# SonyResearch/micro_diffusion

Hardware: AMD Instinct MI355X
Metric: training images/sec (global batch 2048) MicroDiT-XL/2 256-res mask=0.75 (higher is better)
Workload: dtype bf16; 1 GPU; MicroDiT_XL_2 res_256_pretrain.yaml mask=0.75, full step = 2 microbatches x 1024 fwd+bwd + grad exchange + clip 0.25 + AdamW; global_batch=2048, microbatch=1024, parallelism=dp1, grad_exchange=none (single rank)

## Files before the change

### micro_diffusion_amd/csrc/gemm.hip

```cpp
#include "md_common.h"
#include "gemm_common.h"
#include <stdlib.h>

namespace {

constexpr int BM = 128, BN = 128;
constexpr int PITCH_KC = (BKT + 8) * 2;
constexpr int PITCH_KS = (BM + 32) * 2;
constexpr int TILE_BYTES = (BM * PITCH_KC > BKT * PITCH_KS) ? BM * PITCH_KC : BKT * PITCH_KS;
constexpr int SLAB_PITCH = 68;
constexpr int SLAB_FLOATS = 32 * SLAB_PITCH;
static_assert(4 * SLAB_FLOATS * 4 <= 2 * TILE_BYTES, "epilogue slab must fit in the staging LDS");

typedef __attribute__((address_space(3))) s16x4 lds_s16x4;

__device__ __forceinline__ bf16x4 lds_tr_read(const unsigned char* p) {
    s16x4 v = __builtin_amdgcn_ds_read_tr16_b64_v4i16((lds_s16x4*)(p));
    U64 t;
    t.s = v;
    return t.h;
}

__device__ __forceinline__ void tile_coords(int bid, int nwg, int ntn, int group_n, int& tm, int& tn) {
    const int q = nwg >> 3, r = nwg & 7, xcd = bid & 7, j = bid >> 3;
// ... 531 lines not shown
            w4 = md_gemm_w4_fills(t * a->ksplit, a->cu_limit);
        }
        if (a->chosen_variant) *a->chosen_variant = w4 ? MD_GEMM_W4 : MD_GEMM_PP256;
        return w4 ? md_gemm_w4_launch(a, stream) : md_gemm_pp_launch(a, stream);
    }
    if (!a->A || !a->B || !a->C) return MD_BAD_ARG;
    if (a->M <= 0 || a->N <= 0 || a->K <= 0 || a->batch <= 0 || a->ksplit <= 0) return MD_BAD_ARG;
    if (a->lda % 8 || a->ldb % 8) return MD_BAD_ARG;
    if ((a->mode == MD_EPI_STORE_BF16 || a->mode == MD_EPI_RESIDUAL || a->mode == MD_EPI_DACT || a->mode == MD_EPI_SWIGLU_BWD) ? (a->ldc % 8) : (a->ldc % 4))
        return MD_BAD_ARG;
    if (a->C2 && a->ldc2 % 8) return MD_BAD_ARG;
    if (a->ksplit > 1 && !(a->mode == MD_EPI_ATOMIC_F32 || (a->mode == MD_EPI_STORE_F32 && a->sSplit > 0))) return MD_BAD_ARG;
    if (a->mode == MD_EPI_RESIDUAL && (!a->res || (a->gate && a->rows_per_sample <= 0))) return MD_BAD_ARG;
    if (a->mode == MD_EPI_DACT && !a->aux) return MD_BAD_ARG;
    if (a->mode < MD_EPI_STORE_BF16 || a->mode > MD_EPI_SWIGLU_BWD) return MD_BAD_ARG;
    if (a->mode == MD_EPI_SWIGLU_BWD) {
        if (!a->aux || a->ldaux % 8) return MD_BAD_ARG;
        if (a->variant != MD_GEMM_AUTO && a->variant != MD_GEMM_W4) return MD_NOT_ELIGIBLE;
        if (!md_gemm_w4_eligible(a) || (a->cu_limit > 0 && a->cu_limit < 256) || getenv("MD_GEMM_NO_W4")) return MD_NOT_ELIGIBLE;
        a_copy.variant = MD_GEMM_W4;
    }
    if (a->dact_cached && (a->act != MD_ACT_GELU_ERF || !(a->mode == MD_EPI_DACT || (a->mode == MD_EPI_STORE_BF16 && a->C2)))) return MD_BAD_ARG;
    const int64_t tiles256 = ((a->M + 255) / 256) * ((a->N + 255) / 256) * (int64_t)a->batch * a->ksplit;
    const int64_t kspan = (a->K + a->ksplit - 1) / a->ksplit;
    int variant = a->variant;
    if (variant < MD_GEMM_AUTO || variant > MD_GEMM_W4) return MD_BAD_ARG;
    if (variant == MD_GEMM_PP256 && !md_gemm_pp_eligible(a)) return MD_NOT_ELIGIBLE;
    if (variant == MD_GEMM_W4 && !md_gemm_w4_eligible(a)) return MD_NOT_ELIGIBLE;
    if ((a->A_list || a->B_list) && !(a->A_list && a->B_list && md_gemm_pp_eligible(a))) return MD_BAD_ARG;
    if (a->A_list) variant = MD_GEMM_PP256;
    if (variant == MD_GEMM_AUTO) {
        const char* w4min = getenv("MD_GEMM_W4_MIN_TILES");
        if (md_gemm_w4_eligible(a) && tiles256 >= (w4min ? atoi(w4min) : 192) && md_gemm_w4_fills(tiles256, a->cu_limit) && !getenv("MD_GEMM_NO_W4") &&
            (a->a_kcontig || !getenv("MD_GEMM_NO_W4_TN")))
            variant = MD_GEMM_W4;
        else if (md_gemm_pp_eligible(a) && tiles256 >= 192)
            variant = MD_GEMM_PP256;
        else if (!a->a_kcontig && !a->b_kcontig && kspan >= 2048 && tiles256 >= 128)
            variant = MD_GEMM_PACED256;
        else if (a->K >= 1024 && tiles256 >= 224 && tiles256 <= 256)
            variant = MD_GEMM_PACED256;
        else if (kspan > 2048 && tiles256 >= 240 && (tiles256 % 256 == 0 || tiles256 % 256 >= 160 || tiles256 >= 2048))
            variant = MD_GEMM_PACED256;
        else if (a->a_kcontig && a->K <= 2048)
            variant = MD_GEMM_REG128;
        else
            variant = ((!a->a_kcontig && !a->b_kcontig) || a->K < 1024) ? MD_GEMM_REG128 : MD_GEMM_DMA128;
// ... 32 lines not shown
```

### micro_diffusion_amd/csrc/gemm_pp.hip

```cpp
#include "gemm_pp_common.h"

namespace {

constexpr bool pp_is_dact(int epi) { return epi == PP_E_DACT_GELU || epi == PP_E_DACT_MUL; }
constexpr bool pp_is_gelu(int epi) { return epi == PP_E_BF16_GELU || epi == PP_E_BF16_GELU_D; }

template <int EPI>
__device__ __forceinline__ int epi_prefetch_count(const md_gemm_args& p) {
    if (EPI == PP_E_RES) return p.gate ? 5 : 4;
    if (pp_is_dact(EPI)) return 4;
    return 0;
}

template <int EPI, int IH, int JH>
__device__ __forceinline__ void epi_prefetch(const md_gemm_args& p, const PPPlan& w, const EpiTile& et, u32x4 (&pre)[5],
                                             const EpiLane& el) {
    const unsigned ld = EPI == PP_E_RES ? (unsigned)p.ldr : (unsigned)p.ldaux;
    const int mlast = w.M - 1 - et.m0;
    const int nlast = ((w.N - 1) & ~7) - et.n0;
    int rq, cq;
    el.quad_coords(rq, cq);
    const int c = cq + JH * 128;
    const unsigned coff = (unsigned)(c < nlast ? c : nlast);
#pragma unroll
// ... 168 lines not shown
template <int AKC, int BKC, int EPI>
__global__ __launch_bounds__(512) void gemm_bf16_pp_kernel(md_gemm_args p, PPPlan w) {
    __shared__ __attribute__((aligned(1024))) unsigned char smem[2 * B_REGION];
    const int tid = threadIdx.x, lane = tid & 63;
    const int wave = __builtin_amdgcn_readfirstlane(tid >> 6);
    const int wr = wave >> 2, wc = wave & 3;

    constexpr bool TAILABLE = EPI != PP_E_F32;
    int w_first, w_stride, w_count;
    {
        const int G = gridDim.x, x = blockIdx.x & 7, j = blockIdx.x >> 3;
        const int body = (TAILABLE && w.tail_units) ? w.tail_first : w.total;
        const int q = body >> 3, r = body & 7;
        const int lo = x < r ? x * (q + 1) : r * (q + 1) + (x - r) * q;
        const int cnt = q + (x < r ? 1 : 0);
        w_stride = (G - x + 7) >> 3;
        w_first = lo + j;
        w_count = j < cnt ? (int)((unsigned)(cnt - j + w_stride - 1) / (unsigned)w_stride) : 0;
    }
    const int tail_n = (TAILABLE && (int)blockIdx.x < w.tail_units) ? w_count : -1;
    if (w_count == 0 && tail_n < 0) return;
    long long* const tl = p.timeline ? static_cast<long long*>(p.timeline) + (size_t)blockIdx.x * 16 : nullptr;
    if (tl && tid == 0) { tl[0] = clock64(); tl[1] = wall_clock64(); }
    const int half_iters = w_count * (w.nk >> 1) + (tail_n >= 0 ? (w.tail_nk >> 1) : 0);

    const unsigned lds0 = (unsigned)(uintptr_t)(lds_void_t*)smem;
    unsigned adA[4], adB[4];
    frag_addrs<AKC>(adA, lds0, wr * 64, lane);
    frag_addrs<BKC>(adB, lds0 + B_REGION, wc * 32, lane);
    constexpr bool GROUPABLE = !AKC && !BKC && EPI == PP_E_F32;
    int64_t a_kstep = AKC ? (int64_t)BKT * 2 : (int64_t)BKT * w.lda * 2;
    int64_t b_kstep = BKC ? (int64_t)BKT * 2 : (int64_t)BKT * w.ldb * 2;
    const EpiLane el = {lane, wr * 64, wc * 32};

    int s_n = 0, s_kt = 0;
    bool s_live = true;
    const char *sA = nullptr, *sB = nullptr;
    unsigned aofs[2][2], bofs[2][2];
    int s_m0 = 0, s_n0 = 0, s_li = 0, s_seg_kt = 0;
    auto stager_segment = [&](int li) {
        const bf16* Ab = reinterpret_cast<const bf16*>(p.A_list[li]);
        const bf16* Bb = reinterpret_cast<const bf16*>(p.B_list[li]);
        sA = reinterpret_cast<const char*>(AKC ? Ab + (int64_t)s_m0 * w.lda : Ab + s_m0);
        sB = reinterpret_cast<const char*>(BKC ? Bb + (int64_t)s_n0 * w.ldb : Bb + s_n0);
        s_seg_kt = w.nk_seg;
    };
    auto stager_open = [&](int n) {
        int m0, n0, batch, split;
        if (GROUPABLE && w.nprob) {
            int q;
            work_decode_grouped(w, w_first + n * w_stride, q, m0, n0, split);
            const PPProblem& pr = w.prob[q];
            stage_offsets<AKC>(aofs, m0, pr.M, pr.lda, wave, lane);
            stage_offsets<BKC>(bofs, n0, pr.N, pr.ldb, wave, lane);
            a_kstep = (int64_t)BKT * pr.lda * 2;
            b_kstep = (int64_t)BKT * pr.ldb * 2;
            const int64_t kb = (int64_t)split * w.kspan;
            sA = reinterpret_cast<const char*>(reinterpret_cast<const bf16*>(pr.A) + kb * pr.lda + m0);
            sB = reinterpret_cast<const char*>(reinterpret_cast<const bf16*>(pr.B) + kb * pr.ldb + n0);
            return;
        }
        int item = w_first + n * w_stride, ksub = 0;
        if (TAILABLE && n == tail_n) {
            const unsigned u = blockIdx.x, t = u / (unsigned)w.tail_split;
            item = w.tail_first + (int)t;
            ksub = (int)(u - t * (unsigned)w.tail_split) * w.tail_nk * BKT;
        }
        work_decode(w, item, m0, n0, batch, split);
        stage_offsets<AKC>(aofs, m0, w.M, w.lda, wave, lane);
        stage_offsets<BKC>(bofs, n0, w.N, w.ldb, wave, lane);
        if (EPI == PP_E_F32 && p.A_list) {
            s_m0 = m0;
            s_n0 = n0;
            s_li = __builtin_amdgcn_readfirstlane((batch * w.ksplit + split) * w.nseg);
            stager_segment(s_li);
            return;
        }
        const int64_t kbeg = (int64_t)split * w.kspan + ksub;
        const bf16* Ab = reinterpret_cast<const bf16*>(p.A) + (int64_t)batch * p.sA;
        const bf16* Bb = reinterpret_cast<const bf16*>(p.B) + (int64_t)batch * p.sB;
        sA = reinterpret_cast<const char*>(AKC ? Ab + (int64_t)m0 * w.lda + kbeg : Ab + kbeg * w.lda + m0);
        sB = reinterpret_cast<const char*>(BKC ? Bb + (int64_t)n0 * w.ldb + kbeg : Bb + kbeg * w.ldb + n0);
    };
    auto stager_advance = [&]() {
        sA += a_kstep;
        sB += b_kstep;
        if (++s_kt == ((TAILABLE && s_n == tail_n) ? w.tail_nk : w.nk)) {
            s_kt = 0;
            if (++s_n < w_count + (tail_n >= 0 ? 1 : 0)) stager_open(s_n);
            else s_live = false;
        } else if (EPI == PP_E_F32 && p.A_list && --s_seg_kt == 0) {
            stager_segment(++s_li);
        }
    };
#define PP_STAGE(KIND, BUF)                                                                                             \
    do {                                                                                                                \
        if (s_live) {                                                                                                   \
            if (KIND == 0) stage_half(sA, aofs[0], smem + (BUF) * 32768, wave);                                         \
            else if (KIND == 1) stage_half(sB, bofs[0], smem + B_REGION + (BUF) * 32768, wave);                         \
            else if (KIND == 2) stage_half(sB, bofs[1], smem + B_REGION + (BUF) * 32768 + HT, wave);                    \
            else { stage_half(sA, aofs[1], smem + (BUF) * 32768 + HT, wave); stager_advance(); }                        \
        }                                                                                                               \
    } while (0)

    int c_n = 0, c_kt = 0;
    bool epi_pending = false;
    int pf_after = 0;
    EpiTile et = {0, 0, 0, 0, 0, 0, 0, 0, false, nullptr, nullptr, nullptr, nullptr};
    const f32x16 zero16 = {0.f, 0.f, 0.f, 0.f, 0.f, 0.f, 0.f, 0.f, 0.f, 0.f, 0.f, 0.f, 0.f, 0.f, 0.f, 0.f};
    constexpr bool PLAIN_ONLY = EPI == PP_E_RES || pp_is_dact(EPI);
    const int npf = epi_prefetch_count<EPI>(p);
    const bool has_ops = npf > 0;
    u32x4 pre[5];
#pragma unroll
    for (int x = 0; x < 5; ++x) pre[x] = u32x4{0u, 0u, 0u, 0u};

    f32x16 acc[4][2];
#pragma unroll
    for (int q = 0; q < 4; ++q)
#pragma unroll
        for (int i = 0; i < 2; ++i)
#pragma unroll
            for (int r = 0; r < 16; ++r) acc[q][i][r] = 0.f;
    Frag<AKC> fa[2][4];
    Frag<BKC> fb0[4], fb1[4];

    stager_open(0);
    PP_STAGE(0, 0); PP_STAGE(1, 0); PP_STAGE(2, 0); PP_STAGE(3, 0);
// ... 58 lines not shown
#define PP_RAW_WAIT(EPI_PHASE)                                                                                          \
    do {                                                                                                                \
        if (!((EPI_PHASE) && has_ops && epi_was)) {                                                                     \
            if (!s_live) PP_VMCNT(0);                                                                                   \
            else PP_VMCNT(8);                                                                                           \
        }                                                                                                               \
    } while (0)
#define PP_PIN_NONE() do { } while (0)
#define PP_COMPUTE(Q, FB, PINS, FRESH)                                                                                       \
    do {                                                                                                                \
        __builtin_amdgcn_s_barrier();                                                                                   \
        asm volatile("s_waitcnt lgkmcnt(0)" ::: "memory");                                                              \
        PINS;                                                                                                           \
        __builtin_amdgcn_sched_barrier(0);                                                                              \
        __builtin_amdgcn_s_setprio(1);                                                                                  \
        PP_MFMA(Q, FB, FRESH);                                                                                          \
        __builtin_amdgcn_s_setprio(0);                                                                                  \
        __builtin_amdgcn_sched_barrier(0);                                                                              \
        __builtin_amdgcn_s_barrier();                                                                                   \
    } while (0)

    for (int it = 0; it < half_iters; ++it) {
        const bool tail_item = TAILABLE && c_n == tail_n;
        const bool last_pair = (c_kt + 2 == (tail_item ? w.tail_nk : w.nk));
        int kx32 = 32;
        asm volatile("" : "+s"(kx32));
        bool epi_was;
        epi_was = epi_pending;
        PP_EPI(0, 0, 0, 0, 1, true);
        PP_READ_B(fb0, 0, 0); PP_READ_A(0, 0);
        PP_STAGE(2, 1); if (s_live) pf_after = 2;
        PP_RAW_WAIT(true);
        PP_COMPUTE(0, fb0, PP_PIN_B(fb0); PP_PIN_A(), epi_was);
        epi_was = epi_pending;
        PP_EPI(0, 1, 1, 1, 1, true);
        PP_READ_B(fb1, 0, 1);
        { const bool live = s_live; PP_STAGE(3, 1); if (live) pf_after = 2; }
        PP_RAW_WAIT(true);
        PP_COMPUTE(1, fb1, PP_PIN_B(fb1), epi_was);
        epi_was = epi_pending;
        PP_EPI(1, 1, 3, 1, 0, true);
        PP_READ_A(0, 1);
        PP_STAGE(0, 0); if (s_live) pf_after = 2;
        PP_RAW_WAIT(true);
        PP_COMPUTE(3, fb1, PP_PIN_A(), epi_was);
        epi_was = epi_pending;
        PP_EPI(1, 0, 2, 0, 0, false);
// ... 20 lines not shown
            } else {
                work_decode(w, w_first + c_n * w_stride, et.m0, et.n0, et.batch, et.split);
            }
            epi_open<EPI, GROUPABLE>(p, w, et);
            if (has_ops) epi_prefetch<EPI, 0, 0>(p, w, et, pre, el);
        }
        {
            const bool live = s_live;
            PP_STAGE(1, 1);
            pf_after = live ? 2 : 0;
            if (last_pair && has_ops && !tail_item) {
                if (!live) PP_VMCNT(0);
                else if (npf == 5) PP_VMCNT(13);
                else PP_VMCNT(12);
            } else {
                if (live) PP_VMCNT(8); else PP_VMCNT(0);
            }
        }
        PP_COMPUTE(2, fb0, PP_PIN_NONE(), false);
        c_kt += 2;
        if (last_pair) {
            if (tl && tid == 0 && c_n < 8) tl[3 + c_n] = clock64();
            c_kt = 0; ++c_n; epi_pending = true;
        }
    }
    if (wr == 0) __builtin_amdgcn_s_barrier();
    PP_VMCNT(0);
   
#define PP_DRAIN_Q(IH, JH, Q)                                                                                           \
    do {                                                                                                                \
        if (PLAIN_ONLY || et.plain) epi_quadrant<EPI, IH, JH, true>(p, w, acc[Q], et, pre, el);                         \
        else epi_quadrant<EPI, IH, JH, PLAIN_ONLY>(p, w, acc[Q], et, pre, el);                                          \
    } while (0)
#define PP_DRAIN_PF(IH, JH)                                                                                             \
    do {                                                                                                                \
        if (has_ops) {                                                                                                  \
            epi_prefetch<EPI, IH, JH>(p, w, et, pre, el);                                                               \
            PP_VMCNT(0);                                                                                                \
        }                                                                                                               \
    } while (0)
    if (TAILABLE && tail_n >= 0) {
        et.cbase = static_cast<char*>(p.tail_ws) + (size_t)blockIdx.x * (size_t)(PT * PT * 4);
        et.ldc = PT;
        epi_quadrant<PP_E_F32, 0, 0, true>(p, w, acc[0], et, pre, el);
        epi_quadrant<PP_E_F32, 0, 1, true>(p, w, acc[1], et, pre, el);
        epi_quadrant<PP_E_F32, 1, 1, true>(p, w, acc[3], et, pre, el);
// ... 113 lines not shown
            y[i + 1] *= d.y;
        }
        out = make_uint4(cvt_pk_bf16(y[0], y[1]), cvt_pk_bf16(y[2], y[3]), cvt_pk_bf16(y[4], y[5]), cvt_pk_bf16(y[6], y[7]));
    }
    *reinterpret_cast<uint4*>(reinterpret_cast<bf16*>(p.C) + (int64_t)batch * p.sC + (int64_t)gr * p.ldc + gc) = out;
}

}

static bool pp_instantiated(int akc, int bkc, int epi) {
    if (akc && bkc) return epi == PP_E_BF16 || epi == PP_E_RES || epi == PP_E_DACT_GELU || epi == PP_E_DACT_MUL;
    if (akc && !bkc) return epi == PP_E_BF16 || epi == PP_E_BF16_GELU || epi == PP_E_BF16_GELU_D || epi == PP_E_RES || epi == PP_E_F32;
    if (!akc && !bkc) return epi == PP_E_F32;
    return false;
}

bool md_gemm_pp_eligible(const md_gemm_args* a) {
    const int epi = md_gemm_pp_epi_kind(a);
    if (epi < 0 || !pp_instantiated(a->a_kcontig, a->b_kcontig, epi)) return false;
    return md_gemm_pp_shape_ok(a, epi);
}

bool md_gemm_pp_shape_ok(const md_gemm_args* a, int epi) {
    if (a->K % a->ksplit) return false;
    const int64_t kspan = a->K / a->ksplit;
    if (kspan < 128 || kspan % 128) return false;
    if (a->N % 8) return false;
    if ((a->A_list || a->B_list) && epi != PP_E_F32) return false;
    if (a->problems || a->n_problems) {
        if (!a->problems || a->n_problems < 1 || a->n_problems > MD_GEMM_MAX_PROBLEMS) return false;
        if (a->a_kcontig || a->b_kcontig || epi != PP_E_F32 || a->A_list || a->bias || a->alpha != 1.f || a->batch != 1) return false;
        for (int i = 0; i < a->n_problems; ++i) {
            const md_gemm_problem& s = a->problems[i];
            if (!s.A || !s.B || s.M <= 0 || s.N <= 0 || s.N % 8 || s.lda % 8 || s.ldb % 8 || s.c_off % 4 || s.c_off < 0) return false;
            if (s.lda > (1 << 22) || s.ldb > (1 << 22) || s.N > (1 << 20) || s.M >= (1 << 30)) return false;
        }
    }
    if (a->A_list && a->list_segments > 1 && (kspan % ((int64_t)a->list_segments * 128))) return false;
    if (epi == PP_E_RES && a->gate && a->rows_per_sample % 64) return false;
    if ((epi == PP_E_RES || pp_is_dact(epi) || epi == PP_E_DACT_SWIGLU) && (a->bias || a->alpha != 1.f || a->M % PT || a->N % PT))
        return false;
    if (a->M >= (1 << 30) || a->N >= (1 << 30) || a->K >= (1 << 30)) return false;
    if (a->lda > (1 << 22) || a->ldb > (1 << 22)) return false;
    if (a->ldc > (1 << 20) || a->ldc2 > (1 << 20) || a->ldr > (1 << 20) || a->ldaux > (1 << 20) || a->ldg > (1 << 20))
        return false;
    return true;
}

static bool md_gemm_pp_plan_tail(const md_gemm_args* a, int epi, int cus, PPPlan* w) {
    if (!a->tail_ws || a->tail_mode == 1 || epi == PP_E_F32 || a->A_list || a->problems || a->timeline) return false;
    const int G = cus & ~7;
    if (G < 8 || w->total <= G) return false;
    const int r = w->total % G;
    if (r == 0 || r * 2 > G) return false;
    const int iters = w->nk >> 1;
    const double tile_us = 3.1 * iters;
    int s = 0;
    double best = a->tail_mode == 2 ? -1e30 : 2.0;
    for (int c = iters; c >= 2; --c) {
        if (iters % c || (int64_t)r * c > G || (int64_t)r * c * (PT * PT * 4) > a->tail_ws_bytes) continue;
        if (a->tail_mode == 2) { s = c; break; }
        const double gain = tile_us * (1.0 - 1.0 / c) - (0.13 * r * c + 6.0);
        if (gain > best) { best = gain; s = c; }
    }
    if (s < 2) return false;
    w->tail_first = w->total - r;
    w->tail_units = r * s;
    w->tail_split = s;
    w->tail_nk = w->nk / s;
    return true;
}

int md_gemm_pp_launch(const md_gemm_args* a, hipStream_t stream) {
// ... 46 lines not shown
```

### micro_diffusion_amd/csrc/gemm_pp_common.h

```cpp
#pragma once
#include "md_common.h"
#include "gemm_common.h"

namespace {

constexpr int PT = 256;
constexpr int HT = 16384;
constexpr int B_REGION = 65536;
constexpr int NUM_CU = 256;

template <int KC>
struct Frag;
template <>
struct Frag<1> {
    bf16x8 v;
    __device__ __forceinline__ bf16x8 get() const { return v; }
};
template <>
struct Frag<0> {
    bf16x4 lo, hi;
    __device__ __forceinline__ bf16x8 get() const {
        bf16x8 f;
        f[0] = lo[0]; f[1] = lo[1]; f[2] = lo[2]; f[3] = lo[3];
        f[4] = hi[0]; f[5] = hi[1]; f[6] = hi[2]; f[7] = hi[3];
// ... 62 lines not shown
                int gc = r0 + h * 128 + c * 8;
                const int last = (rmax - 1) & ~7;
                gc = (gc < last ? gc : last) - r0;
                ofs[h][j] = (unsigned)(kk * ld + gc) * 2u;
            }
        }
}

__device__ __forceinline__ void stage_half(const char* base, const unsigned (&ofs)[2], unsigned char* slot, int wave) {
#pragma unroll
    for (int j = 0; j < 2; ++j)
        __builtin_amdgcn_global_load_lds((glb_void_t*)(base + ofs[j]), (lds_void_t*)(slot + (wave * 2 + j) * 1024), 16, 0, 0);
}

constexpr int PP_MAX_PROB = MD_GEMM_MAX_PROBLEMS;
struct PPProblem {
    const void* A;
    const void* B;
    int64_t c_off;
    int lda, ldb, M, N;
    int ntm, ntn, tile0, group_n;
};

struct PPPlan {
    int ntm, ntn, ntiles, total;
    int nk;
    int kspan;
    int group_n;
    int M, N, ksplit;
    int lda, ldb;
    int rps_shift;
    int nseg, nk_seg;
    int nprob;
    int tail_first, tail_units, tail_split, tail_nk;
    PPProblem prob[PP_MAX_PROB];
};

__device__ __forceinline__ void work_decode(const PPPlan& w, int item, int& m0, int& n0, int& batch, int& split) {
    const unsigned y = (unsigned)item / (unsigned)w.ntiles;
    const unsigned t = (unsigned)item - y * (unsigned)w.ntiles;
    batch = (int)(y / (unsigned)w.ksplit);
    split = (int)(y - (unsigned)batch * (unsigned)w.ksplit);
    const unsigned per_group = (unsigned)(w.group_n * w.ntm);
    const unsigned g = t / per_group, rem = t - g * per_group;
    const int first_n = (int)g * w.group_n;
    const int gn = (w.ntn - first_n) < w.group_n ? (w.ntn - first_n) : w.group_n;
    const unsigned tm = rem / (unsigned)gn;
    m0 = (int)tm * PT;
    n0 = (first_n + (int)(rem - tm * (unsigned)gn)) * PT;
}

__device__ __forceinline__ void work_decode_grouped(const PPPlan& w, int item, int& q, int& m0, int& n0, int& split) {
    const unsigned y = (unsigned)item / (unsigned)w.ntiles;
    const int t = (int)((unsigned)item - y * (unsigned)w.ntiles);
    split = (int)y;
    q = 0;
#pragma unroll 1
    for (int i = 1; i < w.nprob; ++i)
        if (t >= w.prob[i].tile0) q = i;
    const PPProblem& pr = w.prob[q];
    const unsigned tl = (unsigned)(t - pr.tile0);
    const unsigned per_group = (unsigned)(pr.group_n * pr.ntm);
    const unsigned g = tl / per_group, rem = tl - g * per_group;
    const int first_n = (int)g * pr.group_n;
    const int gn = (pr.ntn - first_n) < pr.group_n ? (pr.ntn - first_n) : pr.group_n;
    const unsigned tm = rem / (unsigned)gn;
    m0 = (int)tm * PT;
    n0 = (first_n + (int)(rem - tm * (unsigned)gn)) * PT;
}

enum {
    PP_E_BF16 = 0,
// ... 119 lines not shown
    const uint4 V0 = quad_sel(odd, W[2], quad_mov4<X1>(W[3])), V1 = quad_sel(!odd, W[3], quad_mov4<X1>(W[2]));
    T[0] = quad_sel(hi2, U0, quad_mov4<X2>(V0));
    T[1] = quad_sel(hi2, U1, quad_mov4<X2>(V1));
    T[2] = quad_sel(!hi2, V0, quad_mov4<X2>(U0));
    T[3] = quad_sel(!hi2, V1, quad_mov4<X2>(U1));
}

#define PP_VMCNT(N) asm volatile("s_waitcnt vmcnt(" #N ")" ::: "memory")


inline int md_gemm_pp_epi_kind(const md_gemm_args* a) {
    switch (a->mode) {
        case MD_EPI_STORE_BF16:
            return a->act == MD_ACT_NONE ? PP_E_BF16 : a->act == MD_ACT_GELU_ERF ? ((a->dact_cached && a->C2) ? PP_E_BF16_GELU_D : PP_E_BF16_GELU) : -1;
        case MD_EPI_RESIDUAL: return PP_E_RES;
        case MD_EPI_DACT: return a->act == MD_ACT_GELU_ERF ? (a->dact_cached ? PP_E_DACT_MUL : PP_E_DACT_GELU) : -1;
        case MD_EPI_STORE_F32: return PP_E_F32;
        case MD_EPI_SWIGLU_BWD: return PP_E_DACT_SWIGLU;
        default: return -1;
    }
}


inline bool md_gemm_pp_plan(const md_gemm_args* a, PPPlan* w) {
    w->nprob = 0;
    w->ntm = (int)((a->M + PT - 1) / PT);
    w->ntn = (int)((a->N + PT - 1) / PT);
    w->ntiles = w->ntm * w->ntn;
    if (a->problems && a->n_problems > 0) {
        w->nprob = a->n_problems;
        int t0 = 0;
        const int64_t kspan_ = a->K / a->ksplit;
        for (int i = 0; i < a->n_problems; ++i) {
            const md_gemm_problem& s = a->problems[i];
            PPProblem& d = w->prob[i];
            d.A = s.A; d.B = s.B; d.c_off = s.c_off;
            d.lda = (int)s.lda; d.ldb = (int)s.ldb; d.M = (int)s.M; d.N = (int)s.N;
            d.ntm = (int)((s.M + PT - 1) / PT);
            d.ntn = (int)((s.N + PT - 1) / PT);
            d.tile0 = t0;
            int64_t g = (2 << 20) / (PT * kspan_ * 2);
            if (g < 4) g = 4;
            if (g > d.ntn) g = d.ntn;
            d.group_n = (int)g;
            t0 += d.ntm * d.ntn;
        }
        w->ntiles = t0;
    }
    const int64_t total = (int64_t)w->ntiles * (w->nprob ? 1 : a->batch) * a->ksplit;
    if (total > (1 << 30)) return false;
    w->total = (int)total;
    w->kspan = (int)(a->K / a->ksplit);
    w->nk = w->kspan / BKT;
    w->nseg = (a->A_list && a->list_segments > 1) ? a->list_segments : 1;
    w->nk_seg = w->nk / w->nseg;
    w->group_n = a->raster_group_n > 0 ? a->raster_group_n : 1;
    w->M = (int)a->M;
    w->N = (int)a->N;
    w->ksplit = a->ksplit;
    w->lda = (int)a->lda;
    w->ldb = (int)a->ldb;
    w->tail_first = w->total;
    w->tail_units = w->tail_split = w->tail_nk = 0;
    w->rps_shift = -1;
    if (a->rows_per_sample > 0 && (a->rows_per_sample & (a->rows_per_sample - 1)) == 0) {
        w->rps_shift = 0;
        while (((int64_t)1 << w->rps_shift) < a->rows_per_sample) ++w->rps_shift;
    }
    return true;
}

}
```

### micro_diffusion_amd/csrc/gemm_w4.hip

```cpp
#include "gemm_pp_common.h"

namespace {

struct W4Addr {
    unsigned adA[8];
    unsigned adB[8];
    unsigned aofs[8], bofs[8];
    unsigned ldsw;
};

#ifndef W4_ACC_INC
#define W4_ACC_INC "gemm_w4_acc.inc"
#endif
#include W4_ACC_INC

constexpr int W4_BUF = 32768;
constexpr int W4_BREG = 65536;
constexpr int W4_SLAB = 8192;

constexpr bool w4_is_dact(int epi) { return epi == PP_E_DACT_GELU || epi == PP_E_DACT_MUL || epi == PP_E_DACT_SWIGLU; }



typedef unsigned w4_u32x2 __attribute__((ext_vector_type(2), may_alias));
// ... 242 lines not shown
    W4_F32_STEP(0, 0) W4_F32_STEP(0, 1) W4_F32_STEP(1, 0) W4_F32_STEP(1, 1) W4_F32_STEP(2, 0) W4_F32_STEP(2, 1) W4_F32_STEP(3, 0) W4_F32_STEP(3, 1)
    W4_F32_STEP(4, 0) W4_F32_STEP(4, 1) W4_F32_STEP(5, 0) W4_F32_STEP(5, 1) W4_F32_STEP(6, 0) W4_F32_STEP(6, 1) W4_F32_STEP(7, 0) W4_F32_STEP(7, 1)
#undef W4_F32_STEP
}

template <int AKC, int BKC, int EPI>
__global__ __launch_bounds__(256) __attribute__((amdgpu_num_vgpr(144))) void gemm_bf16_w4_kernel(md_gemm_args p, PPPlan w) {
    __shared__ __attribute__((aligned(1024))) unsigned char smem[2 * W4_BREG + 4 * W4_SLAB];
    const int tid = threadIdx.x, lane = tid & 63;
    const int wave = __builtin_amdgcn_readfirstlane(tid >> 6);
    const int wr = wave >> 1, wc = wave & 1;

    int w_first, w_stride, w_count;
    {
        const int G = gridDim.x, x = blockIdx.x & 7, j = blockIdx.x >> 3;
        const int q = w.total >> 3, r = w.total & 7;
        const int lo = x < r ? x * (q + 1) : r * (q + 1) + (x - r) * q;
        const int cnt = q + (x < r ? 1 : 0);
        w_stride = (G - x + 7) >> 3;
        w_first = lo + j;
        w_count = j < cnt ? (int)((unsigned)(cnt - j + w_stride - 1) / (unsigned)w_stride) : 0;
    }
    if (w_count == 0) return;
    const int pairs = w_count * (w.nk >> 1);

    const unsigned lds0 = (unsigned)(uintptr_t)(lds_void_t*)smem;
    W4Addr ad;
    {
        const int ra = wr * 128 + (lane & 15), rb = wc * 128 + (lane & 15);
#pragma unroll
        for (int ks = 0; ks < 2; ++ks) {
            if (AKC) ad.adA[ks] = lds0 + (unsigned)(ra * 128 + ((((4 * ks + (lane >> 4)) ^ (ra >> 1)) & 7) << 4));
            if (BKC) ad.adB[ks] = lds0 + (unsigned)(W4_BREG + rb * 128 + ((((4 * ks + (lane >> 4)) ^ (rb >> 1)) & 7) << 4));
        }
        if (AKC) {
#pragma unroll
            for (int i = 2; i < 8; ++i) ad.adA[i] = 0;
        } else {
            const int li = lane & 15, g = lane >> 4;
            const int kk = 8 * g + (li >> 2);
            const int swz = ((kk & 3) << 1) | (((kk >> 3) & 1) << 3);
#pragma unroll
            for (int i = 0; i < 8; ++i) {
                const int col = wr * 128 + 16 * i + 4 * (li & 3);
                ad.adA[i] = lds0 + (unsigned)(kk * 512 + ((((col >> 3) ^ swz) & 31) << 4) + ((col >> 2) & 1) * 8);
            }
        }
        if (!BKC) {
            const int li = lane & 15, g = lane >> 4;
            const int kk = 8 * g + (li >> 2);
            const int swz = ((kk & 3) << 1) | (((kk >> 3) & 1) << 3);
#pragma unroll
            for (int j = 0; j < 8; ++j) {
                const int col = wc * 128 + 16 * j + 4 * (li & 3);
                ad.adB[j] = lds0 + (unsigned)(W4_BREG + kk * 512 + ((((col >> 3) ^ swz) & 31) << 4) + ((col >> 2) & 1) * 8);
            }
        } else {
#pragma unroll
            for (int j = 2; j < 8; ++j) ad.adB[j] = 0;
        }
    }
    ad.ldsw = lds0 + (unsigned)wave * 1024u;

    int s_n = 0, s_kt = 0, s_koffA = 0, s_koffB = 0;
    int kstepA = AKC ? BKT * 2 : BKT * w.lda * 2;
    int kstepB = BKC ? BKT * 2 : BKT * w.ldb * 2;
    constexpr bool GROUPABLE = !AKC && !BKC && EPI == PP_E_F32;
    u32x4 rA, rB;
    auto stager_open = [&](int n) {
        int m0, n0, batch, split;
        if (GROUPABLE && w.nprob) {
            int q;
            work_decode_grouped(w, w_first + n * w_stride, q, m0, n0, split);
            const PPProblem& pr = w.prob[q];
            const int sw = (tid >> 5) & 3;
#pragma unroll
            for (int x = 0; x < 8; ++x) {
                const int c8 = ((tid & 31) ^ ((sw << 1) | ((x & 1) << 3))) * 8;
                const int kr = x * 8 + (tid >> 5);
                ad.aofs[x] = (unsigned)(kr * pr.lda + c8) * 2u;
                ad.bofs[x] = (unsigned)(kr * pr.ldb + c8) * 2u;
            }
            kstepA = BKT * pr.lda * 2;
            kstepB = BKT * pr.ldb * 2;
            const int64_t kb = (int64_t)split * w.kspan;
            const uint64_t ua = (uint64_t)(uintptr_t)(reinterpret_cast<const bf16*>(pr.A) + kb * pr.lda + m0);
            const uint64_t ub = (uint64_t)(uintptr_t)(reinterpret_cast<const bf16*>(pr.B) + kb * pr.ldb + n0);
            rA = u32x4{(unsigned)ua, (unsigned)(ua >> 32) & 0xffffu, 0xffffffffu, 0x00020000u};
            rB = u32x4{(unsigned)ub, (unsigned)(ub >> 32) & 0xffffu, 0xffffffffu, 0x00020000u};
            s_koffA = 0;
            s_koffB = 0;
            return;
        }
        work_decode(w, w_first + n * w_stride, m0, n0, batch, split);
        const int c = ((tid & 7) ^ ((tid >> 4) & 7)) * 8;
#pragma unroll
        for (int x = 0; x < 8; ++x) {
            const int row = x * 32 + (tid >> 3);
            if (AKC) {
                int ga = m0 + row;
                ga = (ga < w.M ? ga : w.M - 1) - m0;
                ad.aofs[x] = (unsigned)(ga * w.lda + c) * 2u;
            } else {
                int gc = m0 + ((tid & 31) ^ ((((tid >> 5) & 3) << 1) | ((x & 1) << 3))) * 8;
                const int last = (w.M - 1) & ~7;
                gc = (gc < last ? gc : last) - m0;
                ad.aofs[x] = (unsigned)((x * 8 + (tid >> 5)) * w.lda + gc) * 2u;
            }
            if (BKC) {
                int gb = n0 + row;
                gb = (gb < w.N ? gb : w.N - 1) - n0;
                ad.bofs[x] = (unsigned)(gb * w.ldb + c) * 2u;
            } else {
                int gc = n0 + ((tid & 31) ^ ((((tid >> 5) & 3) << 1) | ((x & 1) << 3))) * 8;
                const int last = (w.N - 1) & ~7;
                gc = (gc < last ? gc : last) - n0;
                ad.bofs[x] = (unsigned)((x * 8 + (tid >> 5)) * w.ldb + gc) * 2u;
            }
        }
        const int64_t kbeg = (int64_t)split * w.kspan;
        const bf16* pa = reinterpret_cast<const bf16*>(p.A) + (int64_t)batch * p.sA + (AKC ? (int64_t)m0 * w.lda + kbeg : kbeg * w.lda + m0);
        const bf16* pb = reinterpret_cast<const bf16*>(p.B) + (int64_t)batch * p.sB + (BKC ? (int64_t)n0 * w.ldb + kbeg : kbeg * w.ldb + n0);
        const uint64_t ua = (uint64_t)(uintptr_t)pa, ub = (uint64_t)(uintptr_t)pb;
        rA = u32x4{(unsigned)ua, (unsigned)(ua >> 32) & 0xffffu, 0xffffffffu, 0x00020000u};
        rB = u32x4{(unsigned)ub, (unsigned)(ub >> 32) & 0xffffu, 0xffffffffu, 0x00020000u};
        s_koffA = 0;
        s_koffB = 0;
    };
    auto stager_pair_done = [&]() {
        s_kt += 2;
        if (s_kt == w.nk) {
            s_kt = 0;
            if (s_n + 1 < w_count) ++s_n;
            stager_open(s_n);
        }
    };
    stager_open(0);
    w4_prologue<AKC, BKC>(ad, rA, rB, 0, 0, kstepA, kstepB);
    s_koffA = 2 * kstepA;
    s_koffB = 2 * kstepB;
    stager_pair_done();
    w4_first_reads<AKC, BKC>(ad);

    int c_n = 0, c_kt = 0;
#define W4_KTILE(BUF, FRESH)                                                                                            \
    do {                                                                                                                \
        w4_h0<AKC, BKC, BUF, FRESH>(ad, rA, rB, s_koffA, s_koffB);                                                      \
        w4_h1<AKC, BKC, BUF, FRESH>(ad, rA, rB, s_koffA, s_koffB);                                                      \
        w4_h2<AKC, BKC, BUF, FRESH>(ad, rA, rB, s_koffA, s_koffB);                                                      \
        s_koffA += kstepA;                                                                                              \
        s_koffB += kstepB;                                                                                              \
        w4_h3<AKC, BKC, BUF>(ad);                                                                                       \
    } while (0)

    for (int it = 0; it < pairs; ++it) {
        if (c_kt == 0) W4_KTILE(0, true);
        else W4_KTILE(0, false);
        W4_KTILE(1, false);
        stager_pair_done();
        c_kt += 2;
        if (c_kt == w.nk) {
            if constexpr (EPI == PP_E_F32) {
                int m0, n0, batch = 0, split;
                float* tile;
                int64_t ldc;
                if (GROUPABLE && w.nprob) {
                    int q;
                    work_decode_grouped(w, w_first + c_n * w_stride, q, m0, n0, split);
                    const PPProblem& pr = w.prob[q];
                    ldc = pr.N;
                    tile = reinterpret_cast<float*>(p.C) + (int64_t)split * p.sSplit + pr.c_off + (int64_t)m0 * ldc + n0;
                } else {
                    work_decode(w, w_first + c_n * w_stride, m0, n0, batch, split);
                    ldc = p.ldc;
                    tile = reinterpret_cast<float*>(p.C) + (int64_t)batch * p.sC + (int64_t)split * p.sSplit + (int64_t)m0 * ldc + n0;
                }
                asm volatile("s_nop 15\n\ts_nop 15");
                w4_epilogue_f32(tile, ldc, wr * 128, wc * 128, lane);
                c_kt = 0;
                ++c_n;
                continue;
            }
            W4Tile et;
            int split;
            work_decode(w, w_first + c_n * w_stride, et.m0, et.n0, et.batch, split);
            et.mlim = w.M - et.m0;
            et.nlim = w.N - et.n0;
            et.cbase = reinterpret_cast<char*>(p.C) + ((int64_t)et.batch * p.sC + (int64_t)et.m0 * p.ldc + et.n0) * 2;
            et.c2base = (!w4_is_dact(EPI) && p.C2) ? reinterpret_cast<char*>(p.C2) + ((int64_t)et.batch * p.sC2 + (int64_t)et.m0 * p.ldc2 + et.n0) * 2 : nullptr;
            et.opbase = EPI == PP_E_RES   ? reinterpret_cast<const char*>(p.res) + ((int64_t)et.m0 * p.ldr + et.n0) * 2
                        : w4_is_dact(EPI) ? reinterpret_cast<const char*>(p.aux) + ((int64_t)et.batch * p.sAux + (int64_t)et.m0 * p.ldaux + et.n0) * 2
                                          : nullptr;
            et.gbase = (EPI == PP_E_RES && p.gate) ? reinterpret_cast<const char*>(p.gate) + (size_t)et.n0 * 2 : nullptr;
            asm volatile("s_nop 15\n\ts_nop 15");
#ifndef W4_X_NOEPI
            unsigned char* const slab = smem + 2 * W4_BREG + wave * W4_SLAB;
            if (et.mlim >= PT && et.nlim >= PT) w4_epilogue<EPI, true>(p, w, et, slab, wr * 128, wc * 128, lane);
            else w4_epilogue<EPI, false>(p, w, et, slab, wr * 128, wc * 128, lane);
#else
            asm volatile("s_waitcnt vmcnt(0)" ::: "memory");
#endif
            c_kt = 0;
            ++c_n;
        }
    }
    asm volatile("s_waitcnt vmcnt(0)" ::: "memory");
}

}

static bool w4_instantiated(int akc, int bkc, int epi) {
    if (!akc) return !bkc && epi == PP_E_F32;
    if (bkc) return epi == PP_E_BF16 || epi == PP_E_RES || epi == PP_E_DACT_GELU || epi == PP_E_DACT_MUL;
    return epi == PP_E_BF16 || epi == PP_E_BF16_GELU || epi == PP_E_BF16_GELU_D || epi == PP_E_RES || epi == PP_E_DACT_SWIGLU;
}

bool md_gemm_w4_eligible(const md_gemm_args* a) {
    const int epi = md_gemm_pp_epi_kind(a);
    if (epi < 0 || !w4_instantiated(a->a_kcontig, a->b_kcontig, epi)) return false;
    if (!md_gemm_pp_shape_ok(a, epi)) return false;
    if (epi == PP_E_DACT_SWIGLU && (!a->aux || a->batch != 1 || a->ldaux < 2 * a->N || a->ldc < 2 * a->N)) return false;
    if (a->A_list || a->B_list || a->timeline) return false;
    if (a->bias || a->alpha != 1.f) return false;
    const int64_t kspan = a->K / a->ksplit;
    if (epi == PP_E_F32) {
        if (a->ksplit > 1 && a->sSplit <= 0) return false;
        if (a->problems) {
            for (int i = 0; i < a->n_problems; ++i) {
                const md_gemm_problem& s = a->problems[i];
                if (s.M % PT || s.N % PT || kspan * (s.lda > s.ldb ? s.lda : s.ldb) >= ((int64_t)1 << 30)) return false;
            }
            return true;
        }
        if (a->M % PT || a->N % PT || a->ldc % 4) return false;
        return kspan * (a->lda > a->ldb ? a->lda : a->ldb) < ((int64_t)1 << 30);
    }
    if (a->ksplit != 1 || a->problems) return false;
    if (!a->b_kcontig && (a->K * a->ldb >= (int64_t)1 << 30)) return false;
    return true;
}

int md_gemm_w4_launch(const md_gemm_args* a, hipStream_t stream) {
    PPPlan w;
    if (!md_gemm_pp_plan(a, &w)) return MD_BAD_ARG;
    const int cus = (a->cu_limit > 0 && a->cu_limit < NUM_CU) ? a->cu_limit : NUM_CU;
    const unsigned G = (unsigned)(w.total < cus ? w.total : cus);
    if (a->tail_used) *a->tail_used = 0;
// ... 22 lines not shown
```

### micro_diffusion_amd/engine.py

```python
from __future__ import annotations

import ctypes
import math
import os
from ctypes import byref
from typing import Dict, List, Optional

import torch

from . import hip
from .arch import BlockPlan, DiTConfig, caption_ffn_hidden, plan_blocks

BF16, F32, I32 = torch.bfloat16, torch.float32, torch.int32
TAIL_WS_BYTES = 256 * 256 * 256 * 4


class Tape:
    pass


class _Arena:
    ALIGN = 256

    def __init__(self, dev):
# ... 245 lines not shown

    def lin_dgrad(self, dy, wname, dx, M, N, K, *, lddy=None, mode=hip.EPI_STORE_BF16, act=0, aux=None, res=None,
                  dyoff=0):
        self._gemm(A=dy.data_ptr() + 2 * dyoff, B=self.S[wname + ".weight"].data_ptr(), C=dx.data_ptr(), aux=_p(aux),
                   res=_p(res), M=M, N=K, K=N, lda=lddy or N, ldb=K, ldc=K, ldaux=K, ldr=K, batch=1, ksplit=1,
                   a_kcontig=1, b_kcontig=0, mode=mode, act=act, alpha=1.0)

    def _fused12(self, pre):
        w1, w2 = self.S.get(pre + ".w1.weight"), self.S.get(pre + ".w2.weight")
        if w1 is None or w2 is None or (pre + ".w1.bias") in self.P:
            return False
        return (w2.data_ptr() == w1.data_ptr() + w1.numel() * 2 and
                self.G[pre + ".w2.weight"].data_ptr() == self.G[pre + ".w1.weight"].data_ptr() + w1.numel() * 4)

    def _ksplit(self, out_rows, out_cols, contraction, batch=1):
        ws_cap = max(1, self.ws.numel() // (out_rows * out_cols * batch))
        t256 = ((out_rows + 255) // 256) * ((out_cols + 255) // 256) * batch
        if getattr(self, "short_k_accum", True) and contraction <= 512 and t256 >= 64:
            return 1
        if contraction % 128 == 0 and out_cols % 8 == 0:
            units = contraction // 128
            out_us = out_rows * out_cols * batch * 4 / 4e6
            best, best_cost = None, None
            for ks in range(1, min(64, ws_cap, units) + 1):
                if units % ks or t256 * ks < getattr(self, "ksplit_min_items", 192):
                    continue
                per_wg = -(-t256 * ks // 256)
                cost = per_wg * (contraction / ks / 64 * 1.9 + 5.0) + (ks + 2) * out_us
                if best_cost is None or cost < best_cost:
                    best, best_cost = ks, cost
            if best is not None:
                return best if best > 1 else -1
        tiles = ((out_rows + 127) // 128) * ((out_cols + 127) // 128) * batch
        ks = max(1, self.wgrad_target_blocks // tiles)
        ks = min(ks, max(1, contraction // 512))
        return max(1, min(ks, ws_cap))

    def gemm_f32_acc(self, *, out_ptr, M, N, K, ldo, batch=1, sOut=0, accumulate=True, **operands):
        ks = self._ksplit(M, N, K, batch)
        via_ws = ks != 1
        if ks == -1:
            ks, via_ws = 1, self.single_slice_ws
        bf_ptr = self._wgrad_bf16_target(out_ptr, M * N * batch if sOut in (0, M * N) and ldo == N else None) if accumulate else None
        if bf_ptr is not None and not via_ws and ldo % 8:
            via_ws = True
        if not via_ws:
            if bf_ptr is not None:
                self._gemm(C=bf_ptr, M=M, N=N, K=K, ldc=ldo, sC=sOut, batch=batch, ksplit=1, mode=hip.EPI_STORE_BF16, act=0, alpha=1.0,
                           **operands)
                return
            self._gemm(C=out_ptr, M=M, N=N, K=K, ldc=ldo, sC=sOut, batch=batch, ksplit=1,
                       mode=hip.EPI_ACCUM_F32 if accumulate else hip.EPI_STORE_F32, act=0, alpha=1.0, **operands)
            return
        if self.splitk_force_pp and self.gemm_prefer == hip.GEMM_AUTO:
            operands = dict(operands, variant=hip.GEMM_PP256)
        self._gemm(C=self.ws.data_ptr(), M=M, N=N, K=K, ldc=N, sC=ks * M * N, sSplit=M * N, batch=batch, ksplit=ks,
                   mode=hip.EPI_STORE_F32, act=0, alpha=1.0, **operands)
        if bf_ptr is not None:
            self._prof("splitk_reduce", M * N * batch * (4.0 * ks + 2), lambda: hip.check(
# ... 29 lines not shown

    def _wgrad_begin(self):
        self._wgroup = [] if self.group_wgrad else None

    def _wgrad_flush(self):
        grp, self._wgroup = self._wgroup, ([] if self._wgroup is not None else None)
        if not grp:
            return
        if len(grp) == 1:
            g = grp[0]
            self.gemm_f32_acc(out_ptr=g["out"], M=g["M"], N=g["N"], K=g["tokens"], ldo=g["N"], A=g["A"], B=g["B"], lda=g["lda"],
                              ldb=g["ldb"], a_kcontig=0, b_kcontig=0)
            return
        grp.sort(key=lambda g: g["out"])
        base = grp[0]["out"]
        span = max(g["out"] + 4 * g["M"] * g["N"] for g in grp) - base
        span_el = span // 4
        tokens = grp[0]["tokens"]
        units = tokens // 128
        t256 = sum(((g["M"] + 255) // 256) * ((g["N"] + 255) // 256) for g in grp)
        out_us = sum(g["M"] * g["N"] for g in grp) * 4 / 4e6
        ws_cap = self.ws.numel() // span_el
        best, best_cost = None, None
        for ks in range(1, min(64, ws_cap, units) + 1):
            if units % ks:
                continue
            per_wg = -(-t256 * ks // 256)
            cost = per_wg * (tokens / ks / 64 * 1.9 + 5.0) + (ks + 2) * out_us
            if t256 * ks < 192:
                cost *= 192.0 / (t256 * ks)
            if best_cost is None or cost < best_cost:
                best, best_cost = ks, cost
        if best is None:
            for g in grp:
                self.gemm_f32_acc(out_ptr=g["out"], M=g["M"], N=g["N"], K=g["tokens"], ldo=g["N"], A=g["A"], B=g["B"], lda=g["lda"],
                                  ldb=g["ldb"], a_kcontig=0, b_kcontig=0)
            return
        ks = best
        probs = (hip.GemmProblem * len(grp))()
        for i, g in enumerate(grp):
            probs[i] = hip.GemmProblem(g["A"], g["B"], g["lda"], g["ldb"], g["M"], g["N"], (g["out"] - base) // 4)
        g0 = grp[0]
        self._gemm(A=g0["A"], B=g0["B"], C=self.ws.data_ptr(), M=g0["M"], N=g0["N"], K=tokens, lda=g0["lda"], ldb=g0["ldb"], ldc=g0["N"],
                   sSplit=span_el, batch=1, ksplit=ks, a_kcontig=0, b_kcontig=0, mode=hip.EPI_STORE_F32, act=0, alpha=1.0,
                   problems=ctypes.addressof(probs), n_problems=len(grp), _problems=grp)
        runs, cur = [], [grp[0]["out"], grp[0]["out"] + 4 * grp[0]["M"] * grp[0]["N"]]
        for g in grp[1:]:
            if g["out"] == cur[1]:
                cur[1] = g["out"] + 4 * g["M"] * g["N"]
            else:
                runs.append(cur)
# ... 763 lines not shown
```

Measured before the change: 2782 images/sec.

## Allow uneven split-K partitions in PP/W4 GEMMs and widen wgrad split search

Split-K no longer has to divide the contraction evenly. Each split now covers a range of 128-wide K units computed per item, so the PP and W4 kernels track a per-item k-tile count for the f32 (split-workspace) epilogue. The host-side split chooser can then consider non-divisor split counts and uses the actually held CU grid in its cost model. The aim is better load balance and occupancy for weight-gradient GEMMs whose token count has few divisors. The cost is extra per-item bookkeeping, and a loop to count pairs when splits are uneven.

```diff
diff --git a/micro_diffusion_amd/csrc/gemm.hip b/micro_diffusion_amd/csrc/gemm.hip
--- a/micro_diffusion_amd/csrc/gemm.hip
+++ b/micro_diffusion_amd/csrc/gemm.hip
@@ -577,7 +577,7 @@
     }
     if (a->dact_cached && (a->act != MD_ACT_GELU_ERF || !(a->mode == MD_EPI_DACT || (a->mode == MD_EPI_STORE_BF16 && a->C2)))) return MD_BAD_ARG;
     const int64_t tiles256 = ((a->M + 255) / 256) * ((a->N + 255) / 256) * (int64_t)a->batch * a->ksplit;
-    const int64_t kspan = (a->K + a->ksplit - 1) / a->ksplit;
+    const int64_t kspan = a->K % 128 == 0 ? (a->K / 128 + a->ksplit - 1) / a->ksplit * 128 : (a->K + a->ksplit - 1) / a->ksplit;
     int variant = a->variant;
     if (variant < MD_GEMM_AUTO || variant > MD_GEMM_W4) return MD_BAD_ARG;
     if (variant == MD_GEMM_PP256 && !md_gemm_pp_eligible(a)) return MD_NOT_ELIGIBLE;
diff --git a/micro_diffusion_amd/csrc/gemm_pp.hip b/micro_diffusion_amd/csrc/gemm_pp.hip
--- a/micro_diffusion_amd/csrc/gemm_pp.hip
+++ b/micro_diffusion_amd/csrc/gemm_pp.hip
@@ -214,7 +214,9 @@
     if (w_count == 0 && tail_n < 0) return;
     long long* const tl = p.timeline ? static_cast<long long*>(p.timeline) + (size_t)blockIdx.x * 16 : nullptr;
     if (tl && tid == 0) { tl[0] = clock64(); tl[1] = wall_clock64(); }
-    const int half_iters = w_count * (w.nk >> 1) + (tail_n >= 0 ? (w.tail_nk >> 1) : 0);
+    constexpr bool UNEVEN = EPI == PP_E_F32;
+    const int half_iters = (UNEVEN ? items_pairs(w, w_first, w_stride, w_count) : w_count * (w.nk >> 1)) +
+                           (tail_n >= 0 ? (w.tail_nk >> 1) : 0);
 
     const unsigned lds0 = (unsigned)(uintptr_t)(lds_void_t*)smem;
     unsigned adA[4], adB[4];
@@ -226,6 +228,7 @@
     const EpiLane el = {lane, wr * 64, wc * 32};
 
     int s_n = 0, s_kt = 0;
+    int s_nk = w.nk;
     bool s_live = true;
     const char *sA = nullptr, *sB = nullptr;
     unsigned aofs[2][2], bofs[2][2];
@@ -247,7 +250,9 @@
             stage_offsets<BKC>(bofs, n0, pr.N, pr.ldb, wave, lane);
             a_kstep = (int64_t)BKT * pr.lda * 2;
             b_kstep = (int64_t)BKT * pr.ldb * 2;
-            const int64_t kb = (int64_t)split * w.kspan;
+            int kb0;
+            split_range(w, split, kb0, s_nk);
+            const int64_t kb = kb0;
             sA = reinterpret_cast<const char*>(reinterpret_cast<const bf16*>(pr.A) + kb * pr.lda + m0);
             sB = reinterpret_cast<const char*>(reinterpret_cast<const bf16*>(pr.B) + kb * pr.ldb + n0);
             return;
@@ -262,13 +267,19 @@
         stage_offsets<AKC>(aofs, m0, w.M, w.lda, wave, lane);
         stage_offsets<BKC>(bofs, n0, w.N, w.ldb, wave, lane);
         if (EPI == PP_E_F32 && p.A_list) {
+            s_nk = w.nk;
             s_m0 = m0;
             s_n0 = n0;
             s_li = __builtin_amdgcn_readfirstlane((batch * w.ksplit + split) * w.nseg);
             stager_segment(s_li);
             return;
         }
-        const int64_t kbeg = (int64_t)split * w.kspan + ksub;
+        int64_t kbeg = (int64_t)split * (w.nk * BKT) + ksub;
+        if (UNEVEN) {
+            int kb0;
+            split_range(w, split, kb0, s_nk);
+            kbeg = kb0;
+        }
         const bf16* Ab = reinterpret_cast<const bf16*>(p.A) + (int64_t)batch * p.sA;
         const bf16* Bb = reinterpret_cast<const bf16*>(p.B) + (int64_t)batch * p.sB;
         sA = reinterpret_cast<const char*>(AKC ? Ab + (int64_t)m0 * w.lda + kbeg : Ab + kbeg * w.lda + m0);
@@ -277,7 +288,7 @@
     auto stager_advance = [&]() {
         sA += a_kstep;
         sB += b_kstep;
-        if (++s_kt == ((TAILABLE && s_n == tail_n) ? w.tail_nk : w.nk)) {
+        if (++s_kt == ((TAILABLE && s_n == tail_n) ? w.tail_nk : UNEVEN ? s_nk : w.nk)) {
             s_kt = 0;
             if (++s_n < w_count + (tail_n >= 0 ? 1 : 0)) stager_open(s_n);
             else s_live = false;
@@ -296,6 +307,7 @@
     } while (0)
 
     int c_n = 0, c_kt = 0;
+    int c_nk = UNEVEN ? item_nk(w, w_first) : w.nk;
     bool epi_pending = false;
     int pf_after = 0;
     EpiTile et = {0, 0, 0, 0, 0, 0, 0, 0, false, nullptr, nullptr, nullptr, nullptr};
@@ -400,7 +412,7 @@
 
     for (int it = 0; it < half_iters; ++it) {
         const bool tail_item = TAILABLE && c_n == tail_n;
-        const bool last_pair = (c_kt + 2 == (tail_item ? w.tail_nk : w.nk));
+        const bool last_pair = (c_kt + 2 == (tail_item ? w.tail_nk : UNEVEN ? c_nk : w.nk));
         int kx32 = 32;
         asm volatile("" : "+s"(kx32));
         bool epi_was;
@@ -467,6 +479,7 @@
         if (last_pair) {
             if (tl && tid == 0 && c_n < 8) tl[3 + c_n] = clock64();
             c_kt = 0; ++c_n; epi_pending = true;
+            if (UNEVEN && c_n < w_count) c_nk = item_nk(w, w_first + c_n * w_stride);
         }
     }
     if (wr == 0) __builtin_amdgcn_s_barrier();
@@ -626,9 +639,12 @@
 }
 
 bool md_gemm_pp_shape_ok(const md_gemm_args* a, int epi) {
-    if (a->K % a->ksplit) return false;
-    const int64_t kspan = a->K / a->ksplit;
-    if (kspan < 128 || kspan % 128) return false;
+    if (a->K % PP_UNIT) return false;
+    const int64_t units = a->K / PP_UNIT;
+    if (a->ksplit < 1 || a->ksplit > units || units * a->ksplit >= ((int64_t)1 << 31)) return false;
+    const bool uniform = units % a->ksplit == 0;
+    const int64_t kspan = md_gemm_pp_longest_split(a);
+    if (!uniform && epi != PP_E_F32) return false;
     if (a->N % 8) return false;
     if ((a->A_list || a->B_list) && epi != PP_E_F32) return false;
     if (a->problems || a->n_problems) {
@@ -640,6 +656,7 @@
             if (s.lda > (1 << 22) || s.ldb > (1 << 22) || s.N > (1 << 20) || s.M >= (1 << 30)) return false;
         }
     }
+    if ((a->A_list || a->B_list) && !uniform) return false;
     if (a->A_list && a->list_segments > 1 && (kspan % ((int64_t)a->list_segments * 128))) return false;
     if (epi == PP_E_RES && a->gate && a->rows_per_sample % 64) return false;
     if ((epi == PP_E_RES || pp_is_dact(epi) || epi == PP_E_DACT_SWIGLU) && (a->bias || a->alpha != 1.f || a->M % PT || a->N % PT))
@@ -652,7 +669,7 @@
 }
 
 static bool md_gemm_pp_plan_tail(const md_gemm_args* a, int epi, int cus, PPPlan* w) {
-    if (!a->tail_ws || a->tail_mode == 1 || epi == PP_E_F32 || a->A_list || a->problems || a->timeline) return false;
+    if (!a->tail_ws || a->tail_mode == 1 || epi == PP_E_F32 || a->A_list || a->problems || a->timeline || a->ksplit != 1) return false;
     const int G = cus & ~7;
     if (G < 8 || w->total <= G) return false;
     const int r = w->total % G;
diff --git a/micro_diffusion_amd/csrc/gemm_pp_common.h b/micro_diffusion_amd/csrc/gemm_pp_common.h
--- a/micro_diffusion_amd/csrc/gemm_pp_common.h
+++ b/micro_diffusion_amd/csrc/gemm_pp_common.h
@@ -108,10 +108,15 @@
     int ntm, ntn, tile0, group_n;
 };
 
+__host__ __device__ __forceinline__ int pp_split_unit0(int units, int ksplit, int s) {
+    return (int)((unsigned)s * (unsigned)units / (unsigned)ksplit);
+}
+constexpr int PP_UNIT = 128;
+
 struct PPPlan {
     int ntm, ntn, ntiles, total;
+    int units;
     int nk;
-    int kspan;
     int group_n;
     int M, N, ksplit;
     int lda, ldb;
@@ -134,6 +139,25 @@
     const unsigned tm = rem / (unsigned)gn;
     m0 = (int)tm * PT;
     n0 = (first_n + (int)(rem - tm * (unsigned)gn)) * PT;
+}
+
+__device__ __forceinline__ void split_range(const PPPlan& w, int split, int& kbeg, int& nk) {
+    const int u0 = pp_split_unit0(w.units, w.ksplit, split), u1 = pp_split_unit0(w.units, w.ksplit, split + 1);
+    kbeg = u0 * PP_UNIT;
+    nk = (u1 - u0) * (PP_UNIT / BKT);
+}
+__device__ __forceinline__ int item_nk(const PPPlan& w, int item) {
+    const unsigned y = (unsigned)item / (unsigned)w.ntiles;
+    int kbeg, nk;
+    split_range(w, (int)(y % (unsigned)w.ksplit), kbeg, nk);
+    return nk;
+}
+__device__ __forceinline__ int items_pairs(const PPPlan& w, int first, int stride, int count) {
+    if (w.units % w.ksplit == 0) return count * (w.nk >> 1);
+    int pairs = 0;
+#pragma unroll 1
+    for (int n = 0; n < count; ++n) pairs += item_nk(w, first + n * stride) >> 1;
+    return pairs;
 }
 
 __device__ __forceinline__ void work_decode_grouped(const PPPlan& w, int item, int& q, int& m0, int& n0, int& split) {
@@ -299,6 +323,11 @@
 }
 
 
+inline int64_t md_gemm_pp_longest_split(const md_gemm_args* a) {
+    const int64_t units = a->K / PP_UNIT;
+    return (units + a->ksplit - 1) / a->ksplit * PP_UNIT;
+}
+
 inline bool md_gemm_pp_plan(const md_gemm_args* a, PPPlan* w) {
     w->nprob = 0;
     w->ntm = (int)((a->M + PT - 1) / PT);
@@ -307,7 +336,7 @@
     if (a->problems && a->n_problems > 0) {
         w->nprob = a->n_problems;
         int t0 = 0;
-        const int64_t kspan_ = a->K / a->ksplit;
+        const int64_t kspan_ = md_gemm_pp_longest_split(a);
         for (int i = 0; i < a->n_problems; ++i) {
             const md_gemm_problem& s = a->problems[i];
             PPProblem& d = w->prob[i];
@@ -327,8 +356,8 @@
     const int64_t total = (int64_t)w->ntiles * (w->nprob ? 1 : a->batch) * a->ksplit;
     if (total > (1 << 30)) return false;
     w->total = (int)total;
-    w->kspan = (int)(a->K / a->ksplit);
-    w->nk = w->kspan / BKT;
+    w->units = (int)(a->K / PP_UNIT);
+    w->nk = (int)(md_gemm_pp_longest_split(a) / BKT);
     w->nseg = (a->A_list && a->list_segments > 1) ? a->list_segments : 1;
     w->nk_seg = w->nk / w->nseg;
     w->group_n = a->raster_group_n > 0 ? a->raster_group_n : 1;
diff --git a/micro_diffusion_amd/csrc/gemm_w4.hip b/micro_diffusion_amd/csrc/gemm_w4.hip
--- a/micro_diffusion_amd/csrc/gemm_w4.hip
+++ b/micro_diffusion_amd/csrc/gemm_w4.hip
@@ -288,7 +288,8 @@
         w_count = j < cnt ? (int)((unsigned)(cnt - j + w_stride - 1) / (unsigned)w_stride) : 0;
     }
     if (w_count == 0) return;
-    const int pairs = w_count * (w.nk >> 1);
+    constexpr bool UNEVEN = EPI == PP_E_F32;
+    const int pairs = UNEVEN ? items_pairs(w, w_first, w_stride, w_count) : w_count * (w.nk >> 1);
 
     const unsigned lds0 = (unsigned)(uintptr_t)(lds_void_t*)smem;
     W4Addr ad;
@@ -329,6 +330,7 @@
     ad.ldsw = lds0 + (unsigned)wave * 1024u;
 
     int s_n = 0, s_kt = 0, s_koffA = 0, s_koffB = 0;
+    int s_nk = w.nk;
     int kstepA = AKC ? BKT * 2 : BKT * w.lda * 2;
     int kstepB = BKC ? BKT * 2 : BKT * w.ldb * 2;
     constexpr bool GROUPABLE = !AKC && !BKC && EPI == PP_E_F32;
@@ -349,7 +351,9 @@
             }
             kstepA = BKT * pr.lda * 2;
             kstepB = BKT * pr.ldb * 2;
-            const int64_t kb = (int64_t)split * w.kspan;
+            int kb0;
+            split_range(w, split, kb0, s_nk);
+            const int64_t kb = kb0;
             const uint64_t ua = (uint64_t)(uintptr_t)(reinterpret_cast<const bf16*>(pr.A) + kb * pr.lda + m0);
             const uint64_t ub = (uint64_t)(uintptr_t)(reinterpret_cast<const bf16*>(pr.B) + kb * pr.ldb + n0);
             rA = u32x4{(unsigned)ua, (unsigned)(ua >> 32) & 0xffffu, 0xffffffffu, 0x00020000u};
@@ -384,7 +388,12 @@
                 ad.bofs[x] = (unsigned)((x * 8 + (tid >> 5)) * w.ldb + gc) * 2u;
             }
         }
-        const int64_t kbeg = (int64_t)split * w.kspan;
+        int64_t kbeg = (int64_t)split * (w.nk * BKT);
+        if (UNEVEN) {
+            int kb0;
+            split_range(w, split, kb0, s_nk);
+            kbeg = kb0;
+        }
         const bf16* pa = reinterpret_cast<const bf16*>(p.A) + (int64_t)batch * p.sA + (AKC ? (int64_t)m0 * w.lda + kbeg : kbeg * w.lda + m0);
         const bf16* pb = reinterpret_cast<const bf16*>(p.B) + (int64_t)batch * p.sB + (BKC ? (int64_t)n0 * w.ldb + kbeg : kbeg * w.ldb + n0);
         const uint64_t ua = (uint64_t)(uintptr_t)pa, ub = (uint64_t)(uintptr_t)pb;
@@ -395,13 +404,14 @@
     };
     auto stager_pair_done = [&]() {
         s_kt += 2;
-        if (s_kt == w.nk) {
+        if (s_kt == (UNEVEN ? s_nk : w.nk)) {
             s_kt = 0;
             if (s_n + 1 < w_count) ++s_n;
             stager_open(s_n);
         }
     };
     stager_open(0);
+    int c_nk = s_nk;
     w4_prologue<AKC, BKC>(ad, rA, rB, 0, 0, kstepA, kstepB);
     s_koffA = 2 * kstepA;
     s_koffB = 2 * kstepB;
@@ -425,7 +435,7 @@
         W4_KTILE(1, false);
         stager_pair_done();
         c_kt += 2;
-        if (c_kt == w.nk) {
+        if (c_kt == (UNEVEN ? c_nk : w.nk)) {
             if constexpr (EPI == PP_E_F32) {
                 int m0, n0, batch = 0, split;
                 float* tile;
@@ -445,6 +455,7 @@
                 w4_epilogue_f32(tile, ldc, wr * 128, wc * 128, lane);
                 c_kt = 0;
                 ++c_n;
+                if (c_n < w_count) c_nk = item_nk(w, w_first + c_n * w_stride);
                 continue;
             }
             W4Tile et;
@@ -488,7 +499,7 @@
     if (epi == PP_E_DACT_SWIGLU && (!a->aux || a->batch != 1 || a->ldaux < 2 * a->N || a->ldc < 2 * a->N)) return false;
     if (a->A_list || a->B_list || a->timeline) return false;
     if (a->bias || a->alpha != 1.f) return false;
-    const int64_t kspan = a->K / a->ksplit;
+    const int64_t kspan = md_gemm_pp_longest_split(a);
     if (epi == PP_E_F32) {
         if (a->ksplit > 1 && a->sSplit <= 0) return false;
         if (a->problems) {
diff --git a/micro_diffusion_amd/engine.py b/micro_diffusion_amd/engine.py
--- a/micro_diffusion_amd/engine.py
+++ b/micro_diffusion_amd/engine.py
@@ -291,11 +291,12 @@
             units = contraction // 128
             out_us = out_rows * out_cols * batch * 4 / 4e6
             best, best_cost = None, None
-            for ks in range(1, min(64, ws_cap, units) + 1):
-                if units % ks or t256 * ks < getattr(self, "ksplit_min_items", 192):
+            grid = DiTEngine._wgrad_grid(self)
+            for ks, item_units in DiTEngine._split_candidates(units, min(64, ws_cap)):
+                if t256 * ks < getattr(self, "ksplit_min_items", 192):
                     continue
-                per_wg = -(-t256 * ks // 256)
-                cost = per_wg * (contraction / ks / 64 * 1.9 + 5.0) + (ks + 2) * out_us
+                per_wg = -(-t256 * ks // grid)
+                cost = per_wg * (item_units * 2 * 1.9 + 5.0) + (ks + 2) * out_us
                 if best_cost is None or cost < best_cost:
                     best, best_cost = ks, cost
             if best is not None:
@@ -304,6 +305,17 @@
         ks = max(1, self.wgrad_target_blocks // tiles)
         ks = min(ks, max(1, contraction // 512))
         return max(1, min(ks, ws_cap))
+
+    @staticmethod
+    def _split_candidates(units, cap):
+        for ks in range(1, min(cap, units) + 1):
+            if units % ks == 0 or units // ks >= 64:
+                yield ks, -(-units // ks)
+
+    def _wgrad_grid(self):
+        fn = getattr(self, "cu_limit_fn", None)
+        held = fn() if fn is not None else 0
+        return held if 0 < held < 256 else 256
 
     def gemm_f32_acc(self, *, out_ptr, M, N, K, ldo, batch=1, sOut=0, accumulate=True, **operands):
         ks = self._ksplit(M, N, K, batch)
@@ -379,11 +391,10 @@
         out_us = sum(g["M"] * g["N"] for g in grp) * 4 / 4e6
         ws_cap = self.ws.numel() // span_el
         best, best_cost = None, None
-        for ks in range(1, min(64, ws_cap, units) + 1):
-            if units % ks:
-                continue
-            per_wg = -(-t256 * ks // 256)
-            cost = per_wg * (tokens / ks / 64 * 1.9 + 5.0) + (ks + 2) * out_us
+        grid = DiTEngine._wgrad_grid(self)
+        for ks, item_units in DiTEngine._split_candidates(units, min(64, ws_cap)):
+            per_wg = -(-t256 * ks // grid)
+            cost = per_wg * (item_units * 2 * 1.9 + 5.0) + (ks + 2) * out_us
             if t256 * ks < 192:
                 cost *= 192.0 / (t256 * ks)
             if best_cost is None or cost < best_cost:
```

After: 2799 images/sec, median of 6. Within noise of the previous version (+0.6%).
